# hydrusvideodeduplicator/hydrus-video-deduplicator

Measured on AMD Instinct MI355X. Metric: hash-pair comparisons/sec, higher is better.
Workload: dtype fp4(e2m1, +-1 image of the hash bits) x fp4 -> f32, exact

## Files before the change

hydrus-video-deduplicator_amd/csrc/hvd_api.cpp:

```cpp
#include <hip/hip_runtime.h>
#include <rccl/rccl.h>
#include <dlfcn.h>

#include <algorithm>
#include <chrono>
#include <cmath>
#include <cstdarg>
#include <cstdio>
#include <cstring>
#include <mutex>
#include <condition_variable>
#include <functional>
#include <new>
#include <string>
#include <thread>
#include <vector>

#include "hvd_hash_host.h"
#include "hvd_internal.h"
#include "../../include/hvd_mi355x_bench.h"

namespace hvdi {

thread_local char g_err[512] = "";
// ... 80 lines not shown
        n = 0;
    }
    *out_n = n;
    return HVD_OK;
}

int hvd_dct_matrix(float* out) {
    if (!out) return fail(HVD_ERR_ARG, "out is NULL");
    hvd::pdq_dct_table_copy(out);
    return HVD_OK;
}

int hvd_dct_matrix_libm(float* out) {
    if (!out) return fail(HVD_ERR_ARG, "out is NULL");
    fill_dct(out);
    return HVD_OK;
}

}

namespace {

int init_context(int idx, int device) {
    const int saved = t_ctx;
    t_ctx = idx;
    struct Restore {
        int v;
        ~Restore() { t_ctx = v; }
    } restore{saved};
    hipDeviceProp_t prop;
    HIP_TRY(hipGetDeviceProperties(&prop, device));
    if (strncmp(prop.gcnArchName, "gfx950", 6) != 0)
        return fail(HVD_ERR_NO_DEVICE, "device %d is %s; this library is built for gfx950 only", device, prop.gcnArchName);
    HIP_TRY(hipSetDevice(device));
    hvd::pdq_dct_table_copy(g.h_dct);
    hipError_t e = hipStreamCreateWithFlags(&g.stream, hipStreamNonBlocking);
    if (e == hipSuccess) e = hipEventCreate(&g.ev0);
    if (e == hipSuccess) e = hipEventCreate(&g.ev1);
    if (e == hipSuccess) e = hipMalloc((void**)&g.d_dct, sizeof g.h_dct);
    if (e == hipSuccess) e = hipMemcpy(g.d_dct, g.h_dct, sizeof g.h_dct, hipMemcpyHostToDevice);
    if (e != hipSuccess) {
        if (g.d_dct) (void)hipFree(g.d_dct);
        if (g.ev1) (void)hipEventDestroy(g.ev1);
        if (g.ev0) (void)hipEventDestroy(g.ev0);
        if (g.stream) (void)hipStreamDestroy(g.stream);
        g.d_dct = nullptr;
        g.ev0 = g.ev1 = nullptr;
        g.stream = nullptr;
        return fail(HVD_ERR_HIP, "hvd_init(%d): %s", device, hipGetErrorString(e));
    }
    g.device = device;
    g.id = idx;
    g.ready = true;
    return HVD_OK;
}

void shutdown_context(int idx) {
    const int saved = t_ctx;
    t_ctx = idx;
    if (g.ready) {
        (void)hipSetDevice(g.device);
        (void)hipStreamSynchronize(g.stream);
        if (g.comm_ready) {
            free_exchange_buffers();
            (void)ncclCommDestroy(g.comm);
            g.comm_ready = false;
        }
        (void)hipFree(g.d_dct);
        (void)hipEventDestroy(g.ev0);
        (void)hipEventDestroy(g.ev1);
        for (hipEvent_t m : g.mark)
            if (m) (void)hipEventDestroy(m);
        (void)hipStreamDestroy(g.stream);
        for (void** p : {&g.m_a, &g.m_b, &g.m_f, &g.m_o})
            if (*p) (void)hipFree(*p);
        for (void* p : g.scr)
            if (p) (void)hipFree(p);
        if (g.m_srv_stream) {
            (void)hipStreamSynchronize(g.m_srv_stream);
            (void)hipStreamDestroy(g.m_srv_stream);
        }
        if (g.m_pin) (void)hipHostFree(g.m_pin);
        if (g.d2h_pin) (void)hipHostFree(g.d2h_pin);
        g.~Ctx();
        new (&g) Ctx();
    }
    t_ctx = saved;
}

int parse_dct_mode(int* out) {
    *out = hvd::g_pdq_dct_mode;
    if (const char* m = getenv("HVD_PDQ_DCT_MODE")) {
        if (!strcmp(m, "fma") || !strcmp(m, "1")) *out = HVD_DCT_FMA;
        else if (!strcmp(m, "strict") || !strcmp(m, "0") || !*m) *out = HVD_DCT_STRICT;
        else return fail(HVD_ERR_ARG, "HVD_PDQ_DCT_MODE=%s: expected strict or fma", m);
    }
    return HVD_OK;
}

}

namespace hvdi {
std::mutex g_comm_mu;
void abort_group_comms() {
    std::lock_guard<std::mutex> lk(g_comm_mu);
    for (int k = 0; k < g_nctx; ++k)
        if (g_ctx[k].comm_ready) {
            g_ctx[k].comm_ready = false;
            (void)ncclCommAbort(g_ctx[k].comm);
        }
}

void form_group_exchange(bool distinct) {
    const int n_devices = g_nctx;
    g_group_rccl = false;
    if (n_devices <= 1) return;
    std::lock_guard<std::mutex> lk(g_comm_mu);
    bool rccl = distinct && !getenv("HVD_GROUP_NO_RCCL");
    if (rccl) {
        ncclComm_t comms[kMaxCtx];
        int devices[kMaxCtx];
        for (int i = 0; i < n_devices; ++i) devices[i] = g_ctx[i].device;
        ncclResult_t r = ncclCommInitAll(comms, n_devices, devices);
        const int saved = t_ctx;
        if (r == ncclSuccess) {
            for (int i = 0; i < n_devices; ++i) {
                g_ctx[i].comm = comms[i];
                g_ctx[i].comm_ready = true;
            }
            for (int i = 0; i < n_devices && rccl; ++i) {
                t_ctx = i;
                (void)hipSetDevice(g.device);
                g.rank = i;
                g.world = n_devices;
                if (!g.x_cnt_in && hipMalloc(&g.x_cnt_in, 16) != hipSuccess) rccl = false;
                if (!g.x_cnt_all && hipMalloc(&g.x_cnt_all, 16 * (size_t)n_devices) != hipSuccess) rccl = false;
            }
        } else {
            rccl = false;
        }
        if (!rccl) {
            for (int i = 0; i < n_devices; ++i)
                if (g_ctx[i].comm_ready) {
                    t_ctx = i;
                    (void)hipSetDevice(g.device);
                    free_exchange_buffers();
                    (void)ncclCommAbort(g.comm);
                    g.comm_ready = false;
                }
            (void)hipGetLastError();
        }
        t_ctx = saved;
    }
    g_group_rccl = rccl;
    for (int i = 0; i < n_devices; ++i) {
        g_ctx[i].host_exchange = !rccl;
        g_ctx[i].rank = i;
        g_ctx[i].world = n_devices;
    }
}

bool group_devices_distinct() {
    for (int i = 0; i < g_nctx; ++i)
        for (int k = 0; k < i; ++k)
            if (g_ctx[k].device == g_ctx[i].device) return false;
    return true;
// ... 151 lines not shown
    o += "], \"group\": [";
    for (int k = 0; k < g_nctx; ++k) add("%s%d", k ? ", " : "", g_ctx[k].device);
    add("], \"group_exchange\": \"%s\", \"peers\": [", g_nctx <= 1 ? "none" : g_group_rccl ? "rccl" : "host");
    std::vector<int> devs;
    for (int k = 0; k < g_nctx; ++k) devs.push_back(g_ctx[k].device);
    if (devs.size() <= 1) {
        devs.clear();
        for (int d = 0; d < ndev && d < 16; ++d) devs.push_back(d);
    }
    bool first = true;
    for (size_t a = 0; a < devs.size(); ++a)
        for (size_t b = 0; b < devs.size(); ++b) {
            if (devs[a] == devs[b]) continue;
            int can = 0;
            uint32_t link = 0, hops = 0;
            if (hipDeviceCanAccessPeer(&can, devs[a], devs[b]) != hipSuccess) (void)hipGetLastError();
            if (hipExtGetLinkTypeAndHopCount(devs[a], devs[b], &link, &hops) != hipSuccess) {
                (void)hipGetLastError();
                link = 0xFFFFFFFFu;
            }
            const char* lname = link == 4 ? "xgmi" : link == 2 ? "pcie" : link == 0xFFFFFFFFu ? "?" : "other";
            add("%s{\"from\": %d, \"to\": %d, \"access\": %d, \"link\": \"%s\", \"link_type\": %d, \"hops\": %u}", first ? "" : ", ",
                devs[a], devs[b], can, lname, (int)link, hops);
            first = false;
        }
    o += "]}";
    snprintf(buf, len, "%s", o.c_str());
    return o.size() < len ? HVD_OK : fail(HVD_ERR_OVERFLOW, "runtime info needs %zu bytes", o.size() + 1);
}

int hvd_shutdown(void) {
    std::lock_guard<std::mutex> lk(g_mu);
    if (g_nctx == 0) return HVD_OK;
    for (int i = 0; i < g_nctx; ++i) shutdown_context(i);
    hvd::stream_release_cache();
    hvd::mfma_release();
    hvd::pdq_release();
    g_nctx = 0;
    g_group_rccl = false;
    t_ctx = 0;
    return HVD_OK;
}


int hvd_dev_malloc(void** out_ptr, size_t bytes) {
    if (int rc = need_ready()) return rc;
    if (!out_ptr) return fail(HVD_ERR_ARG, "out_ptr is NULL");
    HIP_TRY(hipMalloc(out_ptr, bytes ? bytes : 1));
    return HVD_OK;
}

int hvd_host_malloc(void** out_ptr, size_t bytes) {
    if (int rc = need_ready()) return rc;
    if (!out_ptr) return fail(HVD_ERR_ARG, "out_ptr is NULL");
    HIP_TRY(hipHostMalloc(out_ptr, bytes ? bytes : 1, hipHostMallocDefault));
    return HVD_OK;
}

int hvd_host_free(void* h_ptr) {
    if (int rc = need_ready()) return rc;
    if (h_ptr) HIP_TRY(hipHostFree(h_ptr));
    return HVD_OK;
}

int hvd_dev_free(void* d_ptr) {
    if (int rc = need_ready()) return rc;
    if (d_ptr) HIP_TRY(hipFree(d_ptr));
    return HVD_OK;
}

int hvd_dev_memset(void* d_ptr, int value, size_t bytes) {
    if (int rc = need_ready()) return rc;
    HIP_TRY(hipMemsetAsync(d_ptr, value, bytes, g.stream));
    return HVD_OK;
}

int hvd_memcpy_h2d(void* d_dst, const void* src, size_t bytes) {
    if (int rc = need_ready()) return rc;
    HIP_TRY(hipMemcpyAsync(d_dst, src, bytes, hipMemcpyHostToDevice, g.stream));
    HIP_TRY(hipStreamSynchronize(g.stream));
    return HVD_OK;
}

int hvd_memcpy_d2h(void* dst, const void* d_src, size_t bytes) {
    if (int rc = need_ready()) return rc;
    if (bytes != 0 && bytes <= kSmallD2hMax) {
        std::lock_guard<std::mutex> lk(g.d2h_mu);
        if (!g.d2h_pin && !g.d2h_pin_failed && hipHostMalloc(&g.d2h_pin, kSmallD2hMax, hipHostMallocDefault) != hipSuccess) {
            (void)hipGetLastError();
            g.d2h_pin = nullptr;
            g.d2h_pin_failed = true;
        }
        if (g.d2h_pin) {
            HIP_TRY(hipMemcpyAsync(g.d2h_pin, d_src, bytes, hipMemcpyDeviceToHost, g.stream));
            HIP_TRY(hipStreamSynchronize(g.stream));
            memcpy(dst, g.d2h_pin, bytes);
            return HVD_OK;
        }
    }
    HIP_TRY(hipMemcpyAsync(dst, d_src, bytes, hipMemcpyDeviceToHost, g.stream));
    HIP_TRY(hipStreamSynchronize(g.stream));
    return HVD_OK;
}

int hvd_memcpy_d2d(void* d_dst, const void* d_src, size_t bytes) {
    if (int rc = need_ready()) return rc;
    if (bytes) HIP_TRY(hipMemcpyAsync(d_dst, d_src, bytes, hipMemcpyDeviceToDevice, g.stream));
    return HVD_OK;
}

int hvd_dev_sync(void) {
    if (int rc = need_ready()) return rc;
    HIP_TRY(hipStreamSynchronize(g.stream));
    return HVD_OK;
}

int hvd_device_synchronize(void) {
    if (int rc = need_ready()) return rc;
    HIP_TRY(hipDeviceSynchronize());
    return HVD_OK;
}

int hvd_timer_start(void) {
    if (int rc = need_ready()) return rc;
    HIP_TRY(hipEventRecord(g.ev0, g.stream));
    return HVD_OK;
}

int hvd_timer_stop(float* out_ms) {
    if (int rc = need_ready()) return rc;
    if (!out_ms) return fail(HVD_ERR_ARG, "out_ms is NULL");
    HIP_TRY(hipEventRecord(g.ev1, g.stream));
    HIP_TRY(hipEventSynchronize(g.ev1));
    HIP_TRY(hipEventElapsedTime(out_ms, g.ev0, g.ev1));
    return HVD_OK;
}

int hvd_timer_mark(int slot) {
    if (int rc = need_ready()) return rc;
    if (slot < 0 || slot >= 8) return fail(HVD_ERR_ARG, "timer slot %d: 0..7", slot);
    if (!g.mark[slot]) HIP_TRY(hipEventCreate(&g.mark[slot]));
    HIP_TRY(hipEventRecord(g.mark[slot], g.stream));
    return HVD_OK;
}

int hvd_timer_between(int slot_a, int slot_b, float* out_ms) {
    if (int rc = need_ready()) return rc;
    if (!out_ms || slot_a < 0 || slot_a >= 8 || slot_b < 0 || slot_b >= 8) return fail(HVD_ERR_ARG, "timer slots 0..7, out_ms not NULL");
    if (!g.mark[slot_a] || !g.mark[slot_b]) return fail(HVD_ERR_STATE, "hvd_timer_between: a slot was never marked");
    HIP_TRY(hipEventSynchronize(g.mark[slot_b]));
    HIP_TRY(hipEventElapsedTime(out_ms, g.mark[slot_a], g.mark[slot_b]));
    return HVD_OK;
}

int hvd_set_pdq_dct_mode(int mode) {
    if (mode != HVD_DCT_STRICT && mode != HVD_DCT_FMA) return fail(HVD_ERR_ARG, "unknown DCT mode %d", mode);
    hvd::g_pdq_dct_mode = mode;
    return HVD_OK;
}

int hvd_get_pdq_dct_mode(void) { return hvd::g_pdq_dct_mode; }

int hvd_debug_set(const char* key, int value) {
    if (!key) return fail(HVD_ERR_ARG, "key is NULL");
    if (strcmp(key, "pdq_dct_from_lds") == 0) {
        if (value != 0 && value != 2 && value != 3) return fail(HVD_ERR_ARG, "pdq_dct_from_lds: 0 SGPR operands, 2 literals, 3 by batch size");
        hvd::g_pdq_dct_from_lds = value;
        return HVD_OK;
    }
    if (strcmp(key, "pdq_hash_grid") == 0) {
        if (value < 0) return fail(HVD_ERR_ARG, "pdq_hash_grid must not be negative (0 = default)");
        hvd::g_pdq_hash_grid = value;
        return HVD_OK;
    }
// ... 39 lines not shown
        if (value < 0 || value > 2) return fail(HVD_ERR_ARG, "pdq_down512_wave: 0 never, 1 by batch size, 2 always");
        hvd::g_pdq_down512_wave = value;
        return HVD_OK;
    }
    if (strcmp(key, "pdq_down512_strip") == 0) {
        if (value != 0 && value != 32 && value != 64) return fail(HVD_ERR_ARG, "pdq_down512_strip: 0 by batch size, 32, 64");
        hvd::g_pdq_down512_strip = value;
        return HVD_OK;
    }
    if (strcmp(key, "pdq_down512_wave_grid") == 0) {
        if (value < 0) return fail(HVD_ERR_ARG, "pdq_down512_wave_grid must not be negative (0 = default)");
        hvd::g_pdq_down512_wave_grid = value;
        return HVD_OK;
    }
    if (strcmp(key, "vmatch_slots_log2") == 0) {
        if (value != 0 && (value < 4 || value > 30)) return fail(HVD_ERR_ARG, "vmatch_slots_log2: 0 (automatic) or 4..30");
        for (int k = 0; k < g_nctx; ++k) g_ctx[k].v_force_slots_log2 = value;
        return HVD_OK;
    }
    if (strcmp(key, "vmatch_variant") == 0) {
        if (value != 0 && !hvd::mfma_variant_known(value))
            return fail(HVD_ERR_ARG, "vmatch_variant: 0 (default) or an MFMA form: 8, 9, 12, 13 (auto), 18");
        for (int k = 0; k < g_nctx; ++k) g_ctx[k].v_variant = value;
        return HVD_OK;
    }
    if (strcmp(key, "vmatch_bit_order") == 0) {
        if (value < 0 || value > 2) return fail(HVD_ERR_ARG, "vmatch_bit_order: 0 | 1 | 2");
        for (int k = 0; k < std::max(1, g_nctx); ++k) g_ctx[k].v_bit_order = value;
        return HVD_OK;
    }
#ifndef HVD_NO_BENCH_SYMBOLS
    if (strcmp(key, "allpairs_index_fail_ctx") == 0) {
        if (value < 0) return fail(HVD_ERR_ARG, "allpairs_index_fail_ctx: context + 1, or 0 (off)");
        hvd::g_allpairs_index_fail = value;
        return HVD_OK;
    }
    if (strcmp(key, "index_join_wgs") == 0) {
        if (value < 0 || value > (1 << 20)) return fail(HVD_ERR_ARG, "index_join_wgs: 0 (sized by the device) or 1 .. 2^20 workgroups");
        hvd::g_index_join_wgs = value;
        return HVD_OK;
    }
    if (strcmp(key, "index_tile_split") == 0) {
        if (value != 0 && value != 1 && value != 2 && value != 4) return fail(HVD_ERR_ARG, "index_tile_split: 0 (from n and the device) or 1 | 2 | 4");
        hvd::g_index_tile_split = value;
        return HVD_OK;
    }
    if (strcmp(key, "hash_staging_bytes") == 0) {
        if (value != 0 && value < 4096) return fail(HVD_ERR_ARG, "hash_staging_bytes: 0 (the default, 1 GiB) or >= 4096");
        g_hash_staging_bytes = value;
        return HVD_OK;
    }
    if (strcmp(key, "vmatch_fail_rank") == 0) {
        for (int k = 0; k < g_nctx; ++k) g_ctx[k].v_fail_rank = value;
        return HVD_OK;
    }
    if (strcmp(key, "match_seq") == 0) {
        std::lock_guard<std::mutex> lk(g.m_mu);
        g.m_seq = (uint32_t)value;
        if (g.m_pin) __atomic_store_n(reinterpret_cast<volatile int32_t*>(g.m_pin + hvd::match_two_small_limit()) + 2, value, __ATOMIC_RELEASE);
        return HVD_OK;
    }
#endif
    if (strcmp(key, "vmatch_exchange") == 0) {
        if (value < 0 || value > 2) return fail(HVD_ERR_ARG, "vmatch_exchange: 0 iff world > 1, 1 always, 2 never (partial results)");
        for (int k = 0; k < g_nctx; ++k) g_ctx[k].v_exchange_mode = value;
        return HVD_OK;
    }
    if (strcmp(key, "pdq_fused_down512") == 0) {
        hvd::g_pdq_fused_down512 = value != 0;
        return HVD_OK;
    }
    if (strcmp(key, "pdq_fused_rect") == 0) {
        hvd::g_pdq_fused_rect = value != 0;
        return HVD_OK;
    }
    if (strcmp(key, "match_server") == 0) {
        g_match_server = value != 0;
        return HVD_OK;
    }
    if (strcmp(key, "copy_nt") == 0) {
        hvd::stream_set_copy_nt(value);
        return HVD_OK;
    }
    if (strcmp(key, "mfma_clock_reset") == 0) {
        if (int rc = need_ready()) return rc;
        HIP_TRY(hvd::mfma_clock_reset(t_ctx, g.stream));
        return HVD_OK;
    }
    return fail(HVD_ERR_ARG, "unknown debug key %s", key);
}

int hvd_debug_get(const char* key, int* out_value) {
    if (!key || !out_value) return fail(HVD_ERR_ARG, "NULL argument");
    if (strcmp(key, "match_server_ticks") == 0) {
        const size_t small = hvd::match_two_small_limit();
        *out_value = g.m_pin ? reinterpret_cast<volatile int32_t*>(g.m_pin + small)[8] : 0;
        return HVD_OK;
    }
    if (strcmp(key, "copy_nt") == 0) {
        *out_value = hvd::stream_copy_nt_level();
        return HVD_OK;
    }
    if (strcmp(key, "memcpy_d2h_small_max") == 0) {
        *out_value = (int)kSmallD2hMax;
        return HVD_OK;
    }
    {
        const char* hk[3] = {"hasher_us_copy", "hasher_us_submit", "hasher_us_wait"};
        for (int k = 0; k < 3; ++k)
            if (strcmp(key, hk[k]) == 0) {
                *out_value = (int)std::min<long long>(hvd::stream_take_ns(k) / 1000, 0x7FFFFFFF);
                return HVD_OK;
            }
    }
    if (int rc = need_ready()) return rc;
    static const struct {
        const char* key;
        int word;
    } probe_keys[] = {{"mfma_auto_form", hvd::kSelForm},
                      {"mfma_probe_survivors", hvd::kSelSurvivorsLo},
                      {"mfma_probe_survivors_hi", hvd::kSelSurvivorsHi},
                      {"mfma_auto_half", hvd::kSelSelection},
                      {"mfma_probe_survivors_mix", hvd::kSelSurvivorsMix},
                      {"mfma_probe_close", hvd::kSelIdxClose}};
    for (const auto& pk : probe_keys)
        if (strcmp(key, pk.key) == 0) {
            uint32_t* sel = nullptr;
            HIP_TRY(hvd::mfma_select_buffer(t_ctx, &sel));
            uint32_t v[hvd::kSelectWords] = {};
            HIP_TRY(hipMemcpyAsync(v, sel, sizeof(v), hipMemcpyDeviceToHost, g.stream));
            HIP_TRY(hipStreamSynchronize(g.stream));
            *out_value = (int)v[pk.word];
            return HVD_OK;
        }
    if (strcmp(key, "allpairs_index_used") == 0 || strcmp(key, "allpairs_index_kcand") == 0 || strcmp(key, "allpairs_index_cand_lo") == 0 ||
        strcmp(key, "allpairs_index_max_walk") == 0) {
        uint32_t* sel = nullptr;
        HIP_TRY(hvd::mfma_select_buffer(t_ctx, &sel));
        uint32_t v[hvd::kSelectWords] = {};
        HIP_TRY(hipMemcpyAsync(v, sel, sizeof(v), hipMemcpyDeviceToHost, g.stream));
        HIP_TRY(hipStreamSynchronize(g.stream));
        if (key[15] == 'u') {
            *out_value = (int)v[hvd::kSelIdxUsed];
        } else if (key[15] == 'c') {
            *out_value = (int)(v[hvd::kSelIdxCand] & 0x7FFFFFFFu);
        } else if (key[15] == 'm') {
            *out_value = (int)std::min<uint32_t>(v[hvd::kSelIdxMaxWalk], 0x7FFFFFFFu);
        } else {
            const unsigned long long cand = (unsigned long long)v[hvd::kSelIdxCand] | (unsigned long long)v[hvd::kSelIdxCand + 1] << 32;
            *out_value = (int)std::min<unsigned long long>(cand / 1000ull, 0x7FFFFFFFull);
        }
        return HVD_OK;
    }
#ifndef HVD_NO_BENCH_SYMBOLS
    if (strcmp(key, "index_join_wgs") == 0) {
        uint32_t wgs = 0;
        HIP_TRY(hvd::index_join_workgroups(0u, &wgs));
        *out_value = (int)wgs;
        return HVD_OK;
    }
    if (strcmp(key, "match_seq") == 0 || strcmp(key, "match_server_launches") == 0) {
        std::lock_guard<std::mutex> lk(g.m_mu);
        *out_value = key[8] == 'r' ? (int)g.m_launch : (int)g.m_seq;
        return HVD_OK;
    }
#endif
    if (strcmp(key, "vmatch_bit_order_used") == 0) {
        *out_value = g.v_bit_order_used;
        return HVD_OK;
    }
    {
        const char* vk[3] = {"vmatch_us_local", "vmatch_us_exchange", "vmatch_us_fold"};
        for (int k = 0; k < 3; ++k)
            if (strcmp(key, vk[k]) == 0) {
                *out_value = g.v_us[k];
                return HVD_OK;
            }
    }
    if (strcmp(key, "mfma_pass_khz") == 0 || strcmp(key, "mfma_clock_samples") == 0) {
        unsigned long long v[4] = {0, 0, 0, 0};
        HIP_TRY(hvd::mfma_clock_read(t_ctx, g.stream, v));
        if (key[5] == 'c') {
            *out_value = (int)std::min<unsigned long long>(v[2], 0x7FFFFFFFull);
            return HVD_OK;
        }
        int dev = 0, wall_khz = 0;
        HIP_TRY(hipGetDevice(&dev));
// ... 332 lines not shown
```

hydrus-video-deduplicator_amd/csrc/hvd_internal.h:

```cpp
#pragma once
#include <hip/hip_runtime.h>
#include <rccl/rccl.h>

#include <functional>
#include <mutex>
#include <vector>

#include "host_barrier.h"
#include "hvd_kernels.h"

namespace hvdi {

extern thread_local char g_err[512];
int fail(int code, const char* fmt, ...);

#define HIP_TRY(expr)                                                                                    \
    do {                                                                                                 \
        hipError_t e_ = (expr);                                                                          \
        if (e_ != hipSuccess) return hvdi::fail(HVD_ERR_HIP, "%s: %s", #expr, hipGetErrorString(e_));    \
    } while (0)

#define NCCL_TRY(expr)                                                                                   \
    do {                                                                                                 \
        ncclResult_t r_ = (expr);                                                                        \
        if (r_ != ncclSuccess) return hvdi::fail(HVD_ERR_RCCL, "%s: %s", #expr, ncclGetErrorString(r_)); \
    } while (0)

constexpr size_t kSmallD2hMax = 256u * 1024u;

struct Ctx {
    bool ready = false;
    int device = -1;
    int id = 0;
    bool host_exchange = false;
    hipStream_t stream = nullptr;
    hipEvent_t ev0 = nullptr, ev1 = nullptr;
    hipEvent_t mark[8] = {};
    int v_us[3] = {0, 0, 0};
    float* d_dct = nullptr;
    float h_dct[16 * 64];
    bool comm_ready = false;
    ncclComm_t comm = nullptr;
    int rank = 0, world = 1;
    void* x_cnt_in = nullptr;
    void* x_cnt_all = nullptr;
    void* x_send = nullptr;
    void* x_recv = nullptr;
    size_t x_send_cap = 0, x_recv_cap = 0;
    void* m_a = nullptr;
    void* m_b = nullptr;
    void* m_f = nullptr;
    void* m_o = nullptr;
    size_t m_a_cap = 0, m_b_cap = 0, m_f_cap = 0;
    uint8_t* m_pin = nullptr;
    uint32_t m_seq = 0;
    hipStream_t m_srv_stream = nullptr;
    int32_t m_launch = 0;
    std::mutex m_mu;
    void* d2h_pin = nullptr;
    bool d2h_pin_failed = false;
    std::mutex d2h_mu;
    enum Scr {
        S_DB, S_IMG, S_GRP, S_PAIRS, S_DB2, S_IMG2, S_GRP2, S_VIDQ, S_VIDT, S_OFF, S_SET, S_SET2, S_PKEYS, S_PCNT, S_LIST,
        S_LISTALL, S_VOUT, S_FRAMES, S_FSCR, S_HASH, S_QUAL, S_COMPACT, S_COUNTERS, S_BITS, S_BITS2, S_BROWS, S_BCOOC, S_BITS_O, S_BITS2_O,
        S_IMG_O, S_IMG2_O, S_RECTS, S_OFF2, S_POSQ, S_POST, S_APAIRS, S_AOUT, S_ASCR, S_GREC, S_GLEN, S_GSCORE, S_GSCR, S_GLABEL,
        S_GOUT, S_CQUAL, S_SPREAD, S_COLORS, S_CACC, S_WQ, S_WT, S_N
    };
    void* scr[S_N] = {};
    size_t scr_cap[S_N] = {};
    unsigned long long v_pslots = 0;
    int v_exchange_mode = 0;
    int v_fail_rank = 0;
    int v_force_slots_log2 = 0;
    int v_variant = 0;
    int v_bit_order = 1;
    int v_bit_order_used = 0;
    std::recursive_mutex h_mu;
};
constexpr int kMaxCtx = 16;
extern Ctx g_ctx[kMaxCtx];
extern int g_nctx;
extern bool g_group_rccl;
extern bool g_group_was_rccl;
extern thread_local bool t_agreed_exit;
extern int g_match_server;
extern int64_t g_hash_staging_bytes;
extern thread_local int t_ctx;
#define g (hvdi::g_ctx[hvdi::t_ctx])
extern std::mutex g_mu;

using hvd::HostExchange;
extern HostExchange g_hx;
#define HX_BARRIER(W)                                                                                                      \
    do {                                                                                                                   \
        if (!hvdi::g_hx.barrier(W)) return hvdi::fail(HVD_ERR_RCCL, "group exchange abandoned: another context of the group failed"); \
    } while (0)
struct HxGuard : hvd::HxGuard {
    HxGuard() : hvd::HxGuard(g_hx) {}
};

struct DevBuf {
    void* p = nullptr;
    ~DevBuf() {
        if (p) (void)hipFree(p);
    }
    hipError_t alloc(size_t bytes) { return hipMalloc(&p, bytes ? bytes : 1); }
    template <class T>
    T* as() const {
        return reinterpret_cast<T*>(p);
    }
};

int need_ready();
inline bool pair_less(const hvd_pair& x, const hvd_pair& y) { return x.i != y.i ? x.i < y.i : x.j < y.j; }

int run_on_group(const std::function<int(int)>& fn);
void abort_group_comms();

int agree(unsigned long long count, int own_rc, const char* what, std::vector<unsigned long long>& counts);
int allgather_bytes(const void* d_send, void* d_recv, size_t bytes_per_rank);
void free_exchange_buffers();
int grow(void** p, size_t* cap, size_t need);
int scratch(Ctx::Scr id, size_t need, void** out);
#define SCR(id, bytes, ptr)                                                                  \
    do {                                                                                     \
        if (int rc_ = hvdi::scratch(hvdi::Ctx::id, (bytes), (void**)&(ptr))) return rc_;     \
    } while (0)


int packed_hashes(Ctx::Scr slot, const void* d_img, uint32_t n, void** d_bits);

}
```

hydrus-video-deduplicator_amd/csrc/hvd_kernels.h:

```cpp
#pragma once
#include <hip/hip_runtime.h>
#include <stdint.h>

#include "../../include/hvd_mi355x.h"
#include "hvd_devhash.h"
#include "hvd_mfma_forms.h"

namespace hvd {

struct AllPairsArgs {
    const void* d_db;
    const void* d_db_q = nullptr;
    uint32_t n;
    const int32_t* d_group;
    uint32_t max_dist;
    uint32_t rank, world;
    hvd_pair* d_pairs;
    unsigned long long cap;
    unsigned long long* d_count;
    int variant;
    uint32_t col_chunk;
    int ctx_id = 0;
    VideoSink sink = {nullptr, 0, nullptr, nullptr, nullptr};
    bool sync_decide = false;
// ... 135 lines not shown
    uint32_t nums, dens;
    int max_segments, min_band_votes;
    bool rated, segmented;
    bool args_first;
    static AlignMode of(bool rated, bool segmented, int max_segments = 0, int min_band_votes = 1) {
        return {0u, 0u, max_segments, min_band_votes, rated, segmented, rated};
    }
    unsigned kind() const { return (rated ? 2u : 0u) + (segmented ? 1u : 0u); }
    size_t record_bytes() const {
        constexpr size_t bytes[4] = {sizeof(hvd_valign), sizeof(hvd_vsegments), sizeof(hvd_vrate), sizeof(hvd_vrsegments)};
        return bytes[kind()];
    }
    unsigned runs() const { return segmented ? 2u : 1u; }
    bool records16() const { return rated || segmented; }
};

struct AlignOperands {
    const void *hashes_q, *offsets_q;
    int64_t VQ;
    const void *pos_q, *hashes_t, *offsets_t;
    int64_t VT;
    const void *pos_t, *pairs;
    int64_t M;
    int max_dist, slack;
    void* scratch;
    size_t scratch_bytes;
    void* out;
};

size_t alignment_scratch_bytes(const AlignMode& mode, unsigned long long max_bins);
hipError_t launch_alignment(const AlignMode& mode, const AlignOperands& op, hipStream_t s);

constexpr uint32_t rate_list_length(uint32_t nums, uint32_t dens) {
    uint32_t R = 0;
    while (R < (uint32_t)HVD_ALIGN_MAX_RATES && (((nums | dens) >> (4u * R)) & 15u)) ++R;
    if (R < (uint32_t)HVD_ALIGN_MAX_RATES && ((nums | dens) >> (4u * R))) return 0u;
    for (uint32_t r = 0; r < R; ++r) {
        const uint32_t num = (nums >> (4u * r)) & 15u, den = (dens >> (4u * r)) & 15u;
        if (num - 1u >= 8u || den - 1u >= 8u) return 0u;
        for (uint32_t f = 2; f <= 7u; ++f)
            if (num % f == 0u && den % f == 0u) return 0u;
        for (uint32_t q = 0; q < r; ++q)
            if (((nums >> (4u * q)) & 15u) == num && ((dens >> (4u * q)) & 15u) == den) return 0u;
    }
    return R;
}
inline bool pack_rate_list(const int32_t* rates, int n_rates, uint32_t* nums, uint32_t* dens) {
    *nums = *dens = 0u;
    if (!rates || n_rates < 1 || n_rates > HVD_ALIGN_MAX_RATES) return false;
    uint32_t nn = 0, dd = 0;
    for (int r = 0; r < n_rates; ++r) {
        if (rates[2 * r] < 1 || rates[2 * r] > 8 || rates[2 * r + 1] < 1 || rates[2 * r + 1] > 8) return false;
        nn |= (uint32_t)rates[2 * r] << (4 * r);
        dd |= (uint32_t)rates[2 * r + 1] << (4 * r);
    }
    if (rate_list_length(nn, dd) != (uint32_t)n_rates) return false;
    *nums = nn;
    *dens = dd;
    return true;
}

size_t group_scratch_bytes(unsigned long long V);
hipError_t launch_group_edges(const void* d_records, unsigned long long n_records, const unsigned long long* d_record_count,
                              int kind, const long long* d_lengths, uint32_t T, bool is_min, uint32_t V, const uint32_t* d_score,
                              void* d_scratch, int32_t* d_label, hvd_group* d_groups, unsigned long long cap,
                              unsigned long long* d_count, hipStream_t s);

size_t keeper_scratch_bytes(unsigned long long V);
hipError_t launch_keeper_groups(const void* d_records, unsigned long long n_records, const unsigned long long* d_record_count,
                                int kind, const long long* d_lengths, uint32_t T, bool is_min, uint32_t V, const uint32_t* d_score,
                                void* d_scratch, int32_t* d_keeper, hvd_group* d_groups, unsigned long long cap,
                                unsigned long long* d_count, hipStream_t s, long long* rounds, bool* settled);

hipError_t launch_synth_frames64(uint8_t* d_out, long long v0, uint32_t frames_per_video, unsigned long long n_frames,
                                 uint64_t seed, const int32_t* d_copy_of, hipStream_t s);

hipError_t launch_match_two(const uint32_t* d_a, uint32_t na, const uint32_t* d_b, uint32_t nb, uint32_t max_dist,
                            uint32_t* d_tflags, int32_t* d_hits, hipStream_t s);
uint32_t match_two_small_limit();
hipError_t launch_match_server(const uint32_t* ops, int32_t* hdr, uint32_t last, int32_t launch_id, unsigned long long idle_ticks,
                               unsigned long long life_ticks, hipStream_t s);
hipError_t launch_match_two_small(const uint32_t* a, uint32_t na, const uint32_t* b, uint32_t nb, uint32_t max_dist,
                                  int32_t* hits, int32_t seq, hipStream_t s);

extern int g_pdq_dct_from_lds;
void pdq_dct_table_copy(float* out_16x64);
bool pdq_dct_table_matches(const float* host_16x64);
extern int g_pdq_hash_grid;
extern int g_pdq_dct_mode;
extern bool g_pdq_fused_down512;
extern int g_pdq_down512_wave;
extern int g_pdq_down512_wave_grid;
extern int g_pdq_down512_strip;
hipError_t launch_pdq_hash64(const void* d_in, int kind, int64_t n, const float* d_dct, uint8_t* d_hashes,
                             int32_t* d_quality, hipStream_t s);
hipError_t launch_pdq_dihedral64(const void* d_in, int kind, int64_t n, const float* d_dct, uint8_t* d_hashes8,
                                 int32_t* d_quality, hipStream_t s);

size_t pdq_downsample_ws_floats(int h, int w);
size_t pdq_down512_ws_floats(int64_t n);
hipError_t launch_pdq_downsample(const uint8_t* d_frames, int64_t n, int h, int w, int channels, float* d_ws,
                                 float* d_out64, hipStream_t s);
hipError_t launch_pdq_luma64_rgb(const uint8_t* d_frames, int64_t n, float* d_out64, hipStream_t s);

enum class RectKind { Black, Color, Detail };
struct RectRule {
    RectKind kind;
    int level, count;
};
hipError_t launch_content_rects(const RectRule& rule, const int32_t* d_colors, const uint8_t* d_frames, int64_t n, int h, int w,
                                int channels, const long long* d_offsets, uint32_t V, int32_t* d_rects, hipStream_t s);
hipError_t launch_rect_init(int32_t* d_rects, uint32_t V, hipStream_t s);
hipError_t launch_rect_fold(const RectRule& rule, const int32_t* d_colors, const uint8_t* d_frames, int64_t n, int h, int w,
                            int channels, const long long* d_offsets, uint32_t V, int32_t* d_rects, hipStream_t s);
hipError_t launch_rect_finish(int32_t* d_rects, uint32_t V, int h, int w, hipStream_t s);
hipError_t rect_fold_black(const uint8_t* d_frames, int64_t n, int h, int w, int channels, const long long* d_offsets, uint32_t V,
                           int black_level, int min_bright, int32_t* d_rects, hipStream_t s);
hipError_t rect_fold_color(const uint8_t* d_frames, int64_t n, int h, int w, int channels, const long long* d_offsets, uint32_t V,
                           const int32_t* d_colors, int bar_level, int min_bright, int32_t* d_rects, hipStream_t s);
hipError_t rect_fold_detail(const uint8_t* d_frames, int64_t n, int h, int w, int channels, const long long* d_offsets, uint32_t V,
                            int detail_level, int min_detail, int32_t* d_rects, hipStream_t s);
extern bool g_pdq_fused_rect;
constexpr int kDownRectMax = 512;
void launch_down_rect(const uint8_t* d_frames, int64_t n, int h, int w, int channels, const void* d_geom, float* d_out64,
                      hipStream_t s);
size_t pdq_rects_geom_bytes(int64_t n);
hipError_t launch_pdq_downsample_rects(const uint8_t* d_frames, int64_t n, int h, int w, int channels,
                                       const long long* d_offsets, uint32_t V, const int32_t* d_rects, void* d_geom,
                                       float* d_ws, float* d_out64, hipStream_t s);

size_t bar_colors_scratch_bytes(uint32_t V);
hipError_t launch_bar_colors(const uint8_t* d_frames, int64_t n, int h, int w, int channels, const long long* d_offsets,
                             uint32_t V, int bar_level, int32_t* d_acc, int32_t* d_colors, hipStream_t s);

bool crops_valid(const int32_t* crops, int K, int h, int w);
size_t pdq_crops_scratch_bytes(int64_t n, int h, int w, int K);
hipError_t launch_pdq_hash_crops(const uint8_t* d_frames, int64_t n, int h, int w, int channels, const int32_t* crops, int K,
                                 const float* d_dct, void* d_scratch, uint8_t* d_hashes8, int32_t* d_quality,
                                 int32_t* d_crop_quality, hipStream_t s);

}
```

hydrus-video-deduplicator_amd/csrc/k_hamming_index.hip:

```cpp
#include <hip/hip_runtime.h>
#include <stdint.h>

#include <mutex>
#include <type_traits>

#include "hvd_index_dev.h"
#include "hvd_kernels.h"

namespace {

using namespace hvd::index_dev;

constexpr uint32_t kWavePairs = 64;
constexpr uint32_t kXB = 16;
constexpr uint32_t kYS = 4;
static_assert(kYS == 4u && kXB == 16u, "the join packs the masks of two slots, kXB bits each, into a register, and selects among four");
constexpr uint32_t kQueue = 128;
constexpr uint32_t kRun = 4;
constexpr uint32_t kRuns = 16u * 65536u / kRun;

__device__ __forceinline__ uint32_t key_of(const uint32_t w[8], uint32_t b) { return (w[b >> 1] >> (16u * (b & 1u))) & 0xFFFFu; }

__device__ __forceinline__ void load_words(const uint4* __restrict__ db, uint32_t i, uint32_t w[8]) {
    const uint4 h0 = db[(size_t)i * 2u], h1 = db[(size_t)i * 2u + 1u];
// ... 88 lines not shown
#pragma unroll
    for (uint32_t j = 0; j < kPer; ++j) {
        const uint32_t i = blockIdx.x * kTile + j * kTileThreads + tid;
        if (i < n) load_words(db, i, w[j]);
    }
    __syncthreads();
#pragma unroll
    for (uint32_t b = 0; b < kBlocks; ++b) {
#pragma unroll
        for (uint32_t j = 0; j < kPer; ++j) {
            const uint32_t i = blockIdx.x * kTile + j * kTileThreads + tid;
            if (i < n) {
                const uint32_t key = key_of(w[j], b);
                const uint32_t pos = lds_add(&cur[b * 256u + (key >> 8)]);
                if (pos < n) rec[(size_t)b * n + pos] = make_uint2(i, key | key_of(w[j], b ^ 1u) << 16);
            }
        }
    }
}

struct Chunk {
    uint32_t p, b, lo, hi;
    size_t at;
};
__device__ __forceinline__ bool chunk_of(uint32_t c, uint32_t n, uint32_t csz, const uint32_t* __restrict__ ptotal,
                                         const uint32_t* __restrict__ pbase, const uint32_t* __restrict__ pfirst,
                                         const uint32_t* __restrict__ chunk_p, Chunk* q) {
    if (c >= pfirst[kParts]) return false;
    q->p = chunk_p[c];
    const uint32_t total = ptotal[q->p];
    if (orders_whole(total)) return false;
    q->b = q->p >> 8;
    q->lo = (c - pfirst[q->p]) * csz;
    q->hi = min(total, q->lo + csz);
    q->at = (size_t)q->b * n + pbase[q->p];
    return true;
}

__global__ __launch_bounds__(256) void k_index_count(const uint2* __restrict__ rec, uint32_t n, uint32_t csz,
                                                     const uint32_t* __restrict__ ptotal, const uint32_t* __restrict__ pbase,
                                                     const uint32_t* __restrict__ pfirst, const uint32_t* __restrict__ chunk_p,
                                                     uint32_t* __restrict__ ccount, const uint32_t* __restrict__ select) {
    __shared__ uint32_t bins[256];
    if (select[hvd::kSelIdxGate] == 0u) return;
    Chunk q;
    if (!chunk_of(blockIdx.x, n, csz, ptotal, pbase, pfirst, chunk_p, &q)) return;
    const uint32_t tid = threadIdx.x;
    bins[tid] = 0u;
    __syncthreads();
    const uint2* __restrict__ r = rec + q.at;
#pragma unroll 4
    for (uint32_t e = q.lo + tid; e < q.hi; e += 256u) (void)lds_add(&bins[r[e].y & 255u]);
    __syncthreads();
    ccount[(size_t)blockIdx.x * 256u + tid] = bins[tid];
}

__global__ __launch_bounds__(256) void k_index_offsets(uint32_t n, const uint32_t* __restrict__ ptotal, const uint32_t* __restrict__ pbase,
                                                       const uint32_t* __restrict__ pfirst, uint32_t* __restrict__ ccount,
                                                       uint32_t* __restrict__ cnt, uint32_t* __restrict__ off,
                                                       const uint32_t* __restrict__ select) {
    __shared__ uint32_t wsum[4];
    if (select[hvd::kSelIdxGate] == 0u) return;
    if (orders_whole(ptotal[blockIdx.x])) return;
    const uint32_t p = blockIdx.x, b = p >> 8, tid = threadIdx.x, lane = tid & 63u, wave = tid >> 6;
    const uint32_t c0 = pfirst[p], c1 = min(pfirst[p + 1u], kMaxChunks);
    uint32_t total = 0;
    for (uint32_t c = c0; c < c1; ++c) total += ccount[(size_t)c * 256u + tid];
    const uint32_t incl = wave_incl_scan(total, lane);
    if (lane == 63u) wsum[wave] = incl;
    __syncthreads();
    uint32_t pos = pbase[p] + incl - total;
    for (uint32_t w = 0; w < wave; ++w) pos += wsum[w];
    const uint32_t key = (p & 255u) * 256u + tid;
    cnt[b * kKeys + key] = total;
    off[(size_t)b * (kKeys + 1u) + key] = pos;
    if (key == kKeys - 1u) off[(size_t)b * (kKeys + 1u) + kKeys] = n;
    for (uint32_t c = c0; c < c1; ++c) {
        const uint32_t v = ccount[(size_t)c * 256u + tid];
        ccount[(size_t)c * 256u + tid] = pos;
        pos += v;
    }
}

constexpr uint32_t kStatsGrid = 256u;
constexpr uint32_t kStatsThreads = 1024u;
constexpr uint32_t kStatsPer = 2u;

__global__ __launch_bounds__(kStatsThreads) void k_index_stats(const uint32_t* __restrict__ cnt, uint32_t* __restrict__ select,
                                                               const hvd::IndexRule q) {
    if (select[hvd::kSelIdxGate] == 0u) return;
    unsigned long long cand = 0;
    uint32_t mx = 0;
    const uint32_t stride = gridDim.x * kStatsThreads;
    for (uint32_t t0 = blockIdx.x * kStatsThreads + threadIdx.x; t0 < kBlocks * kKeys; t0 += kStatsPer * stride) {
        uint32_t c[kStatsPer], nb[kStatsPer][16];
#pragma unroll
        for (uint32_t k = 0; k < kStatsPer; ++k) {
            const uint32_t t = min(t0 + k * stride, kBlocks * kKeys - 1u);
            const uint32_t u = t & (kKeys - 1u);
            const uint32_t* __restrict__ cb = cnt + (t & ~(kKeys - 1u));
            c[k] = cb[u];
            if (q.r != 0u) {
#pragma unroll
                for (uint32_t s = 0; s < 16u; ++s) nb[k][s] = cb[u ^ (1u << s)];
            }
        }
#pragma unroll
        for (uint32_t k = 0; k < kStatsPer; ++k) {
            const uint32_t t = t0 + k * stride, u = t & (kKeys - 1u);
            if (t >= kBlocks * kKeys) break;
            const unsigned long long cu = c[k];
            unsigned long long ylen = cu;
            cand += cu * (cu - (cu != 0ull)) / 2ull;
            if (q.r != 0u) {
#pragma unroll
                for (uint32_t s = 0; s < 16u; ++s) ylen += ((u >> s) & 1u) == 0u ? nb[k][s] : 0u;
                cand += cu * (ylen - cu);
            }
            mx = max(mx, (uint32_t)min(cu * ylen, 0xFFFFFFFFull));
        }
    }
    for (int off = 32; off > 0; off >>= 1) {
        cand += __shfl_down(cand, off);
        mx = max(mx, (uint32_t)__shfl_down((int)mx, off));
    }
    constexpr uint32_t kWaves = kStatsThreads / 64u;
    __shared__ unsigned long long part[kWaves];
    __shared__ uint32_t partm[kWaves];
    if ((threadIdx.x & 63u) == 0u) {
        part[threadIdx.x >> 6] = cand;
        partm[threadIdx.x >> 6] = mx;
    }
    __syncthreads();
    if (threadIdx.x != 0u) return;
    unsigned long long sum = 0;
    uint32_t m = 0;
#pragma unroll
    for (uint32_t w = 0; w < kWaves; ++w) {
        sum += part[w];
        m = max(m, partm[w]);
    }
    unsigned long long* cand_w = reinterpret_cast<unsigned long long*>(select + hvd::kSelIdxCand);
    unsigned long long seen = 0;
    if (sum) seen += atomicAdd(cand_w, sum);
    if (m) seen += atomicMax(&select[hvd::kSelIdxMaxWalk], m);
    asm volatile("" ::"v"(seen));
    if (atomicAdd(&select[hvd::kSelIdxTicket], 1u) == gridDim.x - 1u) {
        const unsigned long long total = atomicAdd(cand_w, 0ull);
        const uint32_t big = atomicMax(&select[hvd::kSelIdxMaxWalk], 0u);
        const uint32_t form = atomicAdd(&select[0], 0u);
        select[hvd::kSelIdxUsed] = hvd::index_wins(q, (double)total, (double)big, form) ? 1u : 0u;
    }
}

__global__ __launch_bounds__(256) void k_index_place(const uint2* __restrict__ rec, uint32_t n, uint32_t csz,
                                                     const uint32_t* __restrict__ ptotal, const uint32_t* __restrict__ pbase,
                                                     const uint32_t* __restrict__ pfirst, const uint32_t* __restrict__ chunk_p,
                                                     const uint32_t* __restrict__ ccount, uint32_t* __restrict__ hw, uint32_t* __restrict__ rows,
                                                     const uint32_t* __restrict__ select) {
    __shared__ uint32_t cur[256];
    if (select[hvd::kSelIdxUsed] == 0u) return;
    Chunk q;
    if (!chunk_of(blockIdx.x, n, csz, ptotal, pbase, pfirst, chunk_p, &q)) return;
    const uint32_t tid = threadIdx.x;
    cur[tid] = ccount[(size_t)blockIdx.x * 256u + tid];
    __syncthreads();
    const uint2* __restrict__ r = rec + q.at;
    const size_t base = (size_t)q.b * n;
    constexpr uint32_t kU = 4u;
    for (uint32_t e0 = q.lo; e0 < q.hi; e0 += 256u * kU) {
        uint2 rc[kU];
        uint32_t pos[kU];
#pragma unroll
        for (uint32_t u = 0; u < kU; ++u) {
            const uint32_t e = e0 + u * 256u + tid;
            rc[u] = e < q.hi ? r[e] : make_uint2(n, 0u);
        }
#pragma unroll
        for (uint32_t u = 0; u < kU; ++u) pos[u] = rc[u].x < n ? lds_add(&cur[rc[u].y & 255u]) : n;
#pragma unroll
        for (uint32_t u = 0; u < kU; ++u)
            if (pos[u] < n) {
                hw[base + pos[u]] = rc[u].y;
                rows[base + pos[u]] = rc[u].x;
            }
    }
}

typedef uint32_t u32x16 __attribute__((ext_vector_type(16)));
typedef u32x16 u32x16w __attribute__((aligned(4)));
typedef const __attribute__((address_space(4))) uint32_t kxw;
typedef const __attribute__((address_space(4))) u32x16w kx16;

__device__ __forceinline__ uint32_t word_step(uint32_t fails, uint32_t x, uint32_t y, uint32_t kfail) {
    const uint32_t d = (uint32_t)__popc(x ^ y) + kfail;
    return __builtin_amdgcn_alignbit(fails, d, 31u);
}

struct JoinArgs {
    const uint32_t* off;
    const uint32_t* hw;
    const uint32_t* rows;
    const uint4* db;
    uint32_t n;
    const int32_t* group;
    hvd_pair* out;
    unsigned long long cap;
    unsigned long long* count;
    uint32_t max_dist, r, tw, rank, world;
};

// ... 450 lines not shown
```

Measured before the change: 566000 billion.

## Poll small D2H copies via kernel ticket and tile index stats through LDS

Small device-to-host copies now go through a custom kernel that writes straight into coherent pinned host memory and publishes a sequence word, which the host spin-polls instead of paying hipMemcpyAsync plus stream-sync latency. Separately, k_index_stats is restructured so each block owns an 8K-key window held in LDS: near Hamming-1 neighbour counts are read from shared memory and only the far bits hit global memory, with uint4 vector loads. The polling path adds host CPU spinning and an extra kernel launch. The stats rewrite raises LDS use and ties the grid size to the key layout.

Measured after the change: 569600 billion (median of 2 runs). Within noise of the previous version (+0.6%).

```diff
diff --git a/hydrus-video-deduplicator_amd/csrc/hvd_api.cpp b/hydrus-video-deduplicator_amd/csrc/hvd_api.cpp
--- a/hydrus-video-deduplicator_amd/csrc/hvd_api.cpp
+++ b/hydrus-video-deduplicator_amd/csrc/hvd_api.cpp
@@ -186,6 +186,7 @@
         }
         if (g.m_pin) (void)hipHostFree(g.m_pin);
         if (g.d2h_pin) (void)hipHostFree(g.d2h_pin);
+        if (g.d2h_ticket) (void)hipFree(g.d2h_ticket);
         g.~Ctx();
         new (&g) Ctx();
     }
@@ -503,14 +504,55 @@
     return HVD_OK;
 }
 
+constexpr int kD2hQueryUs = 50;
+static int polled_d2h(void* dst, const void* d_src, size_t bytes, bool* done) {
+    *done = false;
+    if (!g.d2h_ticket && !g.d2h_ticket_failed) {
+        if (hipMalloc((void**)&g.d2h_ticket, sizeof(uint32_t)) != hipSuccess ||
+            hipMemsetAsync(g.d2h_ticket, 0, sizeof(uint32_t), g.stream) != hipSuccess) {
+            (void)hipGetLastError();
+            if (g.d2h_ticket) (void)hipFree(g.d2h_ticket);
+            g.d2h_ticket = nullptr;
+            g.d2h_ticket_failed = true;
+        }
+        *reinterpret_cast<volatile uint32_t*>((uint8_t*)g.d2h_pin + kD2hWordAt) = 0u;
+    }
+    if (!g.d2h_ticket) return HVD_OK;
+    if (++g.d2h_seq == 0u) g.d2h_seq = 1u;
+    const uint32_t seq = g.d2h_seq;
+    uint8_t* at = (uint8_t*)g.d2h_pin + ((uintptr_t)d_src & 15u);
+    uint32_t* word = reinterpret_cast<uint32_t*>((uint8_t*)g.d2h_pin + kD2hWordAt);
+    HIP_TRY(hvd::launch_copy_to_host(d_src, (uint32_t)bytes, at, g.d2h_ticket, word, seq, g.stream));
+    auto next = std::chrono::steady_clock::now() + std::chrono::microseconds(kD2hQueryUs);
+    while (__atomic_load_n(word, __ATOMIC_ACQUIRE) != seq) {
+        if (std::chrono::steady_clock::now() < next) continue;
+        const hipError_t e = hipStreamQuery(g.stream);
+        if (e == hipSuccess) {
+            if (__atomic_load_n(word, __ATOMIC_ACQUIRE) == seq) break;
+            return HVD_OK;
+        }
+        if (e != hipErrorNotReady) HIP_TRY(e);
+        (void)hipGetLastError();
+        next = std::chrono::steady_clock::now() + std::chrono::microseconds(kD2hQueryUs);
+    }
+    memcpy(dst, at, bytes);
+    *done = true;
+    return HVD_OK;
+}
+
 int hvd_memcpy_d2h(void* dst, const void* d_src, size_t bytes) {
     if (int rc = need_ready()) return rc;
     if (bytes != 0 && bytes <= kSmallD2hMax) {
         std::lock_guard<std::mutex> lk(g.d2h_mu);
-        if (!g.d2h_pin && !g.d2h_pin_failed && hipHostMalloc(&g.d2h_pin, kSmallD2hMax, hipHostMallocDefault) != hipSuccess) {
+        if (!g.d2h_pin && !g.d2h_pin_failed && hipHostMalloc(&g.d2h_pin, kD2hPinBytes, hipHostMallocCoherent) != hipSuccess) {
             (void)hipGetLastError();
             g.d2h_pin = nullptr;
             g.d2h_pin_failed = true;
+        }
+        if (g.d2h_pin && bytes <= g.d2h_poll_max) {
+            bool done = false;
+            if (int rc = polled_d2h(dst, d_src, bytes, &done)) return rc;
+            if (done) return HVD_OK;
         }
         if (g.d2h_pin) {
             HIP_TRY(hipMemcpyAsync(g.d2h_pin, d_src, bytes, hipMemcpyDeviceToHost, g.stream));
@@ -716,6 +758,12 @@
         hvd::stream_set_copy_nt(value);
         return HVD_OK;
     }
+    if (strcmp(key, "memcpy_d2h_poll_max") == 0) {
+        if (value < 0 || (size_t)value > kSmallD2hMax) return fail(HVD_ERR_ARG, "memcpy_d2h_poll_max=%d out of range [0,%zu]", value, kSmallD2hMax);
+        std::lock_guard<std::mutex> lk(g.d2h_mu);
+        g.d2h_poll_max = (size_t)value;
+        return HVD_OK;
+    }
     if (strcmp(key, "mfma_clock_reset") == 0) {
         if (int rc = need_ready()) return rc;
         HIP_TRY(hvd::mfma_clock_reset(t_ctx, g.stream));
@@ -737,6 +785,10 @@
     }
     if (strcmp(key, "memcpy_d2h_small_max") == 0) {
         *out_value = (int)kSmallD2hMax;
+        return HVD_OK;
+    }
+    if (strcmp(key, "memcpy_d2h_poll_max") == 0) {
+        *out_value = (int)g.d2h_poll_max;
         return HVD_OK;
     }
     {
diff --git a/hydrus-video-deduplicator_amd/csrc/hvd_internal.h b/hydrus-video-deduplicator_amd/csrc/hvd_internal.h
--- a/hydrus-video-deduplicator_amd/csrc/hvd_internal.h
+++ b/hydrus-video-deduplicator_amd/csrc/hvd_internal.h
@@ -27,6 +27,9 @@
     } while (0)
 
 constexpr size_t kSmallD2hMax = 256u * 1024u;
+constexpr size_t kPolledD2hMax = 16u * 1024u;
+constexpr size_t kD2hWordAt = kSmallD2hMax + 64u;
+constexpr size_t kD2hPinBytes = kD2hWordAt + 64u;
 
 struct Ctx {
     bool ready = false;
@@ -60,6 +63,10 @@
     void* d2h_pin = nullptr;
     bool d2h_pin_failed = false;
     std::mutex d2h_mu;
+    uint32_t* d2h_ticket = nullptr;
+    bool d2h_ticket_failed = false;
+    uint32_t d2h_seq = 0;
+    size_t d2h_poll_max = kPolledD2hMax;
     enum Scr {
         S_DB, S_IMG, S_GRP, S_PAIRS, S_DB2, S_IMG2, S_GRP2, S_VIDQ, S_VIDT, S_OFF, S_SET, S_SET2, S_PKEYS, S_PCNT, S_LIST,
         S_LISTALL, S_VOUT, S_FRAMES, S_FSCR, S_HASH, S_QUAL, S_COMPACT, S_COUNTERS, S_BITS, S_BITS2, S_BROWS, S_BCOOC, S_BITS_O, S_BITS2_O,
diff --git a/hydrus-video-deduplicator_amd/csrc/hvd_kernels.h b/hydrus-video-deduplicator_amd/csrc/hvd_kernels.h
--- a/hydrus-video-deduplicator_amd/csrc/hvd_kernels.h
+++ b/hydrus-video-deduplicator_amd/csrc/hvd_kernels.h
@@ -241,6 +241,8 @@
                                unsigned long long life_ticks, hipStream_t s);
 hipError_t launch_match_two_small(const uint32_t* a, uint32_t na, const uint32_t* b, uint32_t nb, uint32_t max_dist,
                                   int32_t* hits, int32_t seq, hipStream_t s);
+hipError_t launch_copy_to_host(const void* d_src, uint32_t bytes, void* h_dst, uint32_t* d_ticket, uint32_t* h_word, uint32_t seq,
+                               hipStream_t s);
 
 extern int g_pdq_dct_from_lds;
 void pdq_dct_table_copy(float* out_16x64);
diff --git a/hydrus-video-deduplicator_amd/csrc/k_d2h_copy.hip b/hydrus-video-deduplicator_amd/csrc/k_d2h_copy.hip
--- /dev/null
+++ b/hydrus-video-deduplicator_amd/csrc/k_d2h_copy.hip
@@ -0,0 +1,48 @@
+#include <hip/hip_runtime.h>
+#include <stdint.h>
+
+#include "hvd_kernels.h"
+
+namespace {
+
+constexpr uint32_t kCopyThreads = 256u;
+constexpr uint32_t kCopyPerWg = 16384u;
+constexpr uint32_t kCopyMaxWgs = 16u;
+
+__global__ __launch_bounds__(kCopyThreads) void k_copy_to_host(const uint8_t* __restrict__ src, uint32_t bytes, uint8_t* __restrict__ dst,
+                                                               uint32_t* __restrict__ ticket, uint32_t* __restrict__ word, uint32_t seq) {
+    const uint32_t tid = threadIdx.x;
+    const uint32_t head = min(bytes, (16u - (uint32_t)((uintptr_t)src & 15u)) & 15u);
+    const uint32_t units = (bytes - head) / 16u, tail = head + 16u * units;
+    const uint4* __restrict__ s4 = reinterpret_cast<const uint4*>(src + head);
+    uint4* __restrict__ d4 = reinterpret_cast<uint4*>(dst + head);
+    const uint32_t stride = gridDim.x * kCopyThreads;
+#pragma unroll 4
+    for (uint32_t k = blockIdx.x * kCopyThreads + tid; k < units; k += stride) d4[k] = s4[k];
+    if (blockIdx.x == 0u) {
+        if (tid < head) dst[tid] = src[tid];
+        if (tail + tid < bytes) dst[tail + tid] = src[tail + tid];
+    }
+    __threadfence_system();
+    __syncthreads();
+    if (tid != 0u) return;
+    if (atomicAdd(ticket, 1u) != gridDim.x - 1u) return;
+    atomicExch(ticket, 0u);
+    __threadfence_system();
+    __hip_atomic_store(word, seq, __ATOMIC_RELEASE, __HIP_MEMORY_SCOPE_SYSTEM);
+}
+
+}
+
+namespace hvd {
+
+hipError_t launch_copy_to_host(const void* d_src, uint32_t bytes, void* h_dst, uint32_t* d_ticket, uint32_t* h_word, uint32_t seq,
+                               hipStream_t s) {
+    if ((((uintptr_t)d_src ^ (uintptr_t)h_dst) & 15u) != 0u) return hipErrorInvalidValue;
+    const uint32_t wgs = min(kCopyMaxWgs, max(1u, (bytes + kCopyPerWg - 1u) / kCopyPerWg));
+    hipLaunchKernelGGL(k_copy_to_host, dim3(wgs), dim3(kCopyThreads), 0, s, (const uint8_t*)d_src, bytes, (uint8_t*)h_dst, d_ticket, h_word,
+                       seq);
+    return hipGetLastError();
+}
+
+}
diff --git a/hydrus-video-deduplicator_amd/csrc/k_hamming_index.hip b/hydrus-video-deduplicator_amd/csrc/k_hamming_index.hip
--- a/hydrus-video-deduplicator_amd/csrc/k_hamming_index.hip
+++ b/hydrus-video-deduplicator_amd/csrc/k_hamming_index.hip
@@ -194,42 +194,63 @@
     }
 }
 
-constexpr uint32_t kStatsGrid = 256u;
+constexpr uint32_t kStatsW = 13u;
+constexpr uint32_t kStatsWin = 1u << kStatsW;
+constexpr uint32_t kStatsGrid = kBlocks * (kKeys >> kStatsW);
 constexpr uint32_t kStatsThreads = 1024u;
-constexpr uint32_t kStatsPer = 2u;
+constexpr uint32_t kStatsQuads = kStatsWin / 4u / kStatsThreads;
+static_assert(kStatsW >= 12u && kStatsW <= 14u, "at least one quad per thread, at most 64 KiB of LDS");
 
 __global__ __launch_bounds__(kStatsThreads) void k_index_stats(const uint32_t* __restrict__ cnt, uint32_t* __restrict__ select,
                                                                const hvd::IndexRule q) {
+    __shared__ uint4 win[kStatsWin / 4u];
     if (select[hvd::kSelIdxGate] == 0u) return;
     unsigned long long cand = 0;
     uint32_t mx = 0;
-    const uint32_t stride = gridDim.x * kStatsThreads;
-    for (uint32_t t0 = blockIdx.x * kStatsThreads + threadIdx.x; t0 < kBlocks * kKeys; t0 += kStatsPer * stride) {
-        uint32_t c[kStatsPer], nb[kStatsPer][16];
-#pragma unroll
-        for (uint32_t k = 0; k < kStatsPer; ++k) {
-            const uint32_t t = min(t0 + k * stride, kBlocks * kKeys - 1u);
-            const uint32_t u = t & (kKeys - 1u);
-            const uint32_t* __restrict__ cb = cnt + (t & ~(kKeys - 1u));
-            c[k] = cb[u];
-            if (q.r != 0u) {
-#pragma unroll
-                for (uint32_t s = 0; s < 16u; ++s) nb[k][s] = cb[u ^ (1u << s)];
-            }
-        }
-#pragma unroll
-        for (uint32_t k = 0; k < kStatsPer; ++k) {
-            const uint32_t t = t0 + k * stride, u = t & (kKeys - 1u);
-            if (t >= kBlocks * kKeys) break;
-            const unsigned long long cu = c[k];
-            unsigned long long ylen = cu;
-            cand += cu * (cu - (cu != 0ull)) / 2ull;
-            if (q.r != 0u) {
-#pragma unroll
-                for (uint32_t s = 0; s < 16u; ++s) ylen += ((u >> s) & 1u) == 0u ? nb[k][s] : 0u;
-                cand += cu * (ylen - cu);
-            }
-            mx = max(mx, (uint32_t)min(cu * ylen, 0xFFFFFFFFull));
+    constexpr uint32_t kFar = 16u - kStatsW, kWins = kKeys >> kStatsW;
+    const uint32_t tid = threadIdx.x, u_win = (blockIdx.x % kWins) << kStatsW;
+    const uint4* __restrict__ cb = reinterpret_cast<const uint4*>(cnt + (blockIdx.x / kWins) * kKeys);
+    uint4 c[kStatsQuads], far[kStatsQuads][kFar];
+#pragma unroll
+    for (uint32_t j = 0; j < kStatsQuads; ++j) {
+        const uint32_t at = u_win / 4u + j * kStatsThreads + tid;
+        c[j] = cb[at];
+        if (q.r != 0u) {
+#pragma unroll
+            for (uint32_t s = 0; s < kFar; ++s) far[j][s] = cb[at ^ (kStatsWin / 4u << s)];
+        }
+    }
+    if (q.r != 0u) {
+#pragma unroll
+        for (uint32_t j = 0; j < kStatsQuads; ++j) win[j * kStatsThreads + tid] = c[j];
+        __syncthreads();
+    }
+#pragma unroll
+    for (uint32_t j = 0; j < kStatsQuads; ++j) {
+        const uint32_t qd = j * kStatsThreads + tid, u0 = u_win + 4u * qd;
+        const uint32_t cu[4] = {c[j].x, c[j].y, c[j].z, c[j].w};
+        unsigned long long up[4] = {0ull, 0ull, 0ull, 0ull};
+        if (q.r != 0u) {
+            up[0] = (unsigned long long)cu[1] + cu[2];
+            up[1] = cu[3];
+            up[2] = cu[3];
+#pragma unroll
+            for (uint32_t s = 2; s < 16u; ++s) {
+                const uint4 v = s < kStatsW ? win[qd ^ (1u << (s - 2u))] : far[j][s < kStatsW ? 0u : s - kStatsW];
+                if (((u0 >> s) & 1u) == 0u) {
+                    up[0] += v.x;
+                    up[1] += v.y;
+                    up[2] += v.z;
+                    up[3] += v.w;
+                }
+            }
+        }
+#pragma unroll
+        for (uint32_t k = 0; k < 4u; ++k) {
+            const unsigned long long ck = cu[k], ylen = ck + up[k];
+            cand += ck * (ck - (ck != 0ull)) / 2ull;
+            cand += ck * (ylen - ck);
+            mx = max(mx, (uint32_t)min(ck * ylen, 0xFFFFFFFFull));
         }
     }
     for (int off = 32; off > 0; off >>= 1) {
@@ -237,8 +258,9 @@
         mx = max(mx, (uint32_t)__shfl_down((int)mx, off));
     }
     constexpr uint32_t kWaves = kStatsThreads / 64u;
-    __shared__ unsigned long long part[kWaves];
-    __shared__ uint32_t partm[kWaves];
+    __syncthreads();
+    unsigned long long* part = reinterpret_cast<unsigned long long*>(win);
+    uint32_t* partm = reinterpret_cast<uint32_t*>(part + kWaves);
     if ((threadIdx.x & 63u) == 0u) {
         part[threadIdx.x >> 6] = cand;
         partm[threadIdx.x >> 6] = mx;
```
